# IBM/mcp-context-forge

Hardware: AMD Instinct MI355X
Metric: tool_call_req_per_s (higher is better)
Workload: dtype bf16

## Files before the change

mcp_context_forge_amd/engine.py:

```python

from __future__ import annotations

import asyncio
import json
import logging
import struct
import time
from typing import Any, Dict, List, Optional

from .config import Settings, get_settings
from .db.engine import Database
from .plugins.framework import PluginManager
from .plugins.loader import default_chain_specs, load_plugin_manager
from .protocol import jsonrpc
from .protocol.mcp import PROTOCOL_VERSION, initialize_result
from .registry.registry import NotFoundError, Registry
from .services.a2a_service import A2AService
from .services.content import CompletionService, PromptService, ResourceService, RootService
from .services.gateway_service import GatewayService
from .services.governance import CatalogService, ContentSecurity, PasswordPolicy, TokenBlocklist
from .services.llm_proxy import LLMProxyError, LLMProxyService
from .services.metrics import MetricsBuffer
from .services.observability import AuditTrail, ComplianceService, ObservabilityService, SiemExporter
from .services.sessions import CancellationService, ElicitationService, SessionRegistry
# ... 109 lines not shown
        interval = max(5.0, min(60.0, self.settings.metrics_buffer_flush_interval))
        while not self._maintenance_stop.is_set():
            try:
                await asyncio.wait_for(self._maintenance_stop.wait(), timeout=interval)
                return
            except asyncio.TimeoutError:
                pass
            try:
                self.metrics.maybe_flush()
                self.token_usage.flush()
                self.sessions.cleanup_expired()
                self.observability.flush()
                self.token_blocklist.purge_expired()
            except Exception:
                logger.exception("maintenance loop error")

    async def shutdown(self) -> None:
        if self._maintenance_task is not None:
            self._maintenance_stop.set()
            self._maintenance_task.cancel()
            try:
                await self._maintenance_task
            except (asyncio.CancelledError, Exception):
                pass
            self._maintenance_task = None
        if self.leader_elector is not None:
            await self.leader_elector.stop()
            self.leader_elector = None
        await self.gateway_service.stop()
        await self.a2a_service.aclose()
        await self.llm_proxy.aclose()
        await self.tool_service.aclose()
        await self.plugins.shutdown()
        self.observability.flush()
        self.metrics.flush()
        self.db.close()

    def enable_gpu(self) -> bool:
        if self.gpu_pipeline is not None:
            return True
        if not self.settings.gpu_enabled:
            return False
        try:
            import torch

            if not torch.cuda.is_available():
                return False
            from .gpu.pipeline import GpuPluginPipeline

            self.gpu_pipeline = GpuPluginPipeline(self)
            return True
        except Exception as exc:
            logger.warning("GPU pipeline unavailable: %s", exc)
            return False

    async def handle_rpc(self, req: jsonrpc.JSONRPCRequest, user: Optional[str] = None,
                         server_id: Optional[str] = None, session: Optional[Any] = None,
                         headers: Optional[Dict[str, str]] = None) -> Optional[jsonrpc.JSONRPCResponse]:
        method = req.method
        params = req.params if isinstance(req.params, dict) else {}
        rid = req.id
        try:
            if method == "initialize":
                if session is not None:
                    session.initialized = True
                    session.protocol_version = params.get("protocolVersion")
# ... 225 lines not shown
```

mcp_context_forge_amd/gpu/classifier.py:

```python

from __future__ import annotations

import torch

from ..models.classifier import HashedTextClassifier
from ..ops import hip


class GpuClassifier:
    def __init__(self, model: HashedTextClassifier, device: str = "cuda"):
        self.dim = model.dim
        self.hidden = model.hidden
        self.classes = model.classes
        assert self.dim % 64 == 0 and self.hidden % 128 == 0, "MFMA tile constraints"
        with torch.no_grad():
            self.w1t = model.w1.t().contiguous().to(device=device, dtype=torch.bfloat16)
            self.b1 = model.b1.to(device=device, dtype=torch.float32).contiguous()
            self.w2t = model.w2.t().contiguous().to(device=device, dtype=torch.bfloat16)
            self.b2 = model.b2.to(device=device, dtype=torch.float32).contiguous()

    def forward(self, feats_bf16: torch.Tensor) -> torch.Tensor:
        h = hip.gemm_bt(feats_bf16, self.w1t, self.b1, act=hip.ACT_GELU, out_bf16=True)
        return hip.gemv_head(h, self.w2t, self.b2, act=hip.ACT_SIGMOID)

    def forward_into(self, feats_bf16: torch.Tensor, h_buf: torch.Tensor,
                     scores_buf: torch.Tensor) -> None:
        hip.gemm_bt(feats_bf16, self.w1t, self.b1, act=hip.ACT_GELU, out_bf16=True, out=h_buf)
        hip.gemv_head(h_buf, self.w2t, self.b2, act=hip.ACT_SIGMOID, out=scores_buf)
```

mcp_context_forge_amd/gpu/pipeline.py:

```python

from __future__ import annotations

import asyncio
import json
import os
import time
import uuid
from typing import Any, Callable, Dict, List, Optional, Tuple

import numpy as np
import torch

from ..models.classifier import category_names
from ..ops import dfa, hip
from ..ops.entropy import TOL as ENTROPY_TOL
from ..ops.pybridge import get as _pb_get
from ..plugins.builtin import PII_PATTERNS, _text_of, _walk_strings
from ..plugins.framework import PluginMode
from ..protocol import jsonrpc
from ..services.upstream import InProcUpstream
from ..utils.jsonschema import validate as _validate
from .batch import pack_texts
from .classifier import GpuClassifier
from .graphs import Pass1Graphs, Pass3Graphs
# ... 73 lines not shown
                dfa.compile_patterns(
                    ["".join(ch if ch.isalnum() else "\\" + ch for ch in t) if not t.startswith("[") else t
                     for t in _NORMALIZE_TRIGGERS], case_insensitive=False), device)

        self._secret_tabs: List[Tuple[torch.Tensor, float]] = []
        if self.secrets is not None:
            tables = self.secrets.scan_tables()
            if tables is not None:
                self.banks["secrets"] = hip.DeviceScanTables(tables, device)
            self._secret_tabs = [(hip.entropy_table(tab, device), thr)
                                 for (_a, _c, tab, thr) in self.secrets.entropy_detectors]
            if not self._secret_tabs:
                self._secret_tabs = [(hip.entropy_table(np.full(256, 0xFF, dtype=np.uint8), device),
                                      float("inf"))]

        self._exfil_kw: Optional[hip.DeviceScanTables] = None
        self._exfil_tabs: List[Tuple[torch.Tensor, int]] = []
        if self.exfil is not None:
            self._exfil_kw = hip.DeviceScanTables(self.exfil.keyword_tables(), device)
            self._exfil_tabs = [(hip.entropy_table(tab, device), bits)
                                for (_e, _c, tab, bits) in self.exfil.detectors]

        self._sql_kw: Optional[hip.DeviceScanTables] = None
        self._sql_kw_len: Optional[torch.Tensor] = None
        if self.sql is not None:
            self._sql_kw = hip.DeviceScanTables(self.sql.keyword_tables(), device)
            self._sql_kw_len = torch.tensor(self.sql.keyword_lengths(), dtype=torch.int32, device=device)

        self.classifier: Optional[GpuClassifier] = None
        self.feat_dim = s.gpu_feature_dim
        if self.moderation is not None:
            self.classifier = GpuClassifier(self.moderation.model, device)
            self.feat_dim = self.moderation.dim

        self.semcache: Optional[GpuSemanticCache] = None
        if self.semcache_plugin is not None and self.semcache_plugin.cacheable_tools:
            self.semcache = GpuSemanticCache(
                capacity=max(128, (s.gpu_semcache_capacity // 128) * 128),
                dim=self.feat_dim,
                threshold=self.semcache_plugin.threshold,
                ttl_s=self.semcache_plugin.ttl,
                device=device,
                sketch_dim=s.gpu_semcache_sketch_dim,
            )

        self._pii_fixed: List[int] = []
        self._pii_active_mask = 0
        if self.pii is not None:
            fixed_index = {n: k for k, (n, _, _) in enumerate(PII_PATTERNS)}
            self._pii_fixed = [fixed_index[a[0]] for a in self.pii.active]
            self._pii_active_mask = sum(1 << i for i in self._pii_fixed)
        words = [w.lower() if self.deny.case_insensitive else w for w in self.deny.words] if self.deny else []
        self._deny_lane_ok = bool(words) and all(w.isascii() for w in words)
        self._deny_lane_blob, self._deny_lane_off = pack_strtable(words) if self._deny_lane_ok else (None, None)
        ph = [p.lower() for p in (getattr(self.harm, "phrases", None) or [])]
        self._harm_lane_ok = all(p.isascii() for p in ph)
        self._harm_lane_blob, self._harm_lane_off = pack_strtable(ph) if ph and self._harm_lane_ok else (None, None)

        self._pb = _pb_get()
        self._gpu_lock = asyncio.Lock()
        self._pin = torch.empty(16 << 20, dtype=torch.uint8, pin_memory=True)
        self._pin_off = 0

        self.banks["postmeta"] = hip.DeviceScanTables(
            dfa.compile_literals(['"structuredContent"'], case_insensitive=False), device)

# ... 319 lines not shown
            if args is BAD_ARGS:
                continue
            errs = self._schema_errors(rs.meta(j), args)
            if errs:
                rs.block(j, msg_schema(errs))
            elif hit[j]:
                rs.answer_cached(j, self._cache_result_bytes(int(hit_slot[j])))
            else:
                extra_py.append((j, args))
        return extra_py

    async def _a2a_fast_invoke(self, mt: _ToolMeta, args: Any) -> Dict[str, Any]:
        message = args.get("message") if isinstance(args, dict) else None
        if not isinstance(message, str):
            message = json.dumps(args or {}, default=str)
        t0 = time.monotonic()
        reply_text = await mt.handler(message, {})
        sc = {"agent": mt.original_name, "response": reply_text,
              "latency_ms": round((time.monotonic() - t0) * 1000, 2),
              "uaid": uuid.uuid4().hex}
        return {"content": [{"type": "text", "text": reply_text}],
                "structuredContent": sc, "isError": False}

    async def _await_gpu(self) -> None:
        ev = torch.cuda.Event()
        ev.record()
        if ev.query():
            return
        for _ in range(200000):
            await asyncio.sleep(0)
            if ev.query():
                return
        await asyncio.to_thread(ev.synchronize)

    def _upload(self, arr: np.ndarray) -> torch.Tensor:
        raw = arr.view(np.uint8).reshape(-1)
        n = raw.nbytes
        off = (self._pin_off + 255) & ~255
        if off + n > self._pin.numel():
            grow = max(self._pin.numel() * 2, off + n)
            self._pin = torch.empty(grow, dtype=torch.uint8, pin_memory=True)
            off = 0
        self._pin_off = off + n
        view = self._pin[off:off + n]
        view.numpy()[:] = raw
        cap = 1 << max(16, (n - 1).bit_length()) if n else 1
        dev = torch.empty(cap, dtype=torch.uint8, device=self.device)[:n]
        dev.copy_(view, non_blocking=True)
        tdt = {np.dtype(np.uint8): torch.uint8, np.dtype(np.int32): torch.int32,
               np.dtype(np.int64): torch.int64, np.dtype(np.float32): torch.float32}[np.dtype(arr.dtype)]
        return dev.view(tdt).reshape(arr.shape)

    async def _scan_pass(self, graphs, bankset, blob: np.ndarray, beg: np.ndarray, end: np.ndarray,
                         m: int, extra: Optional[Callable] = None, timed: bool = False):
        toc = self._toc if timed else (lambda key, t: None)
        t_g = self._tic()
        out = scores = ext = None
        await self._gpu_lock.acquire()
        try:
            toc("gp1_lockwait", t_g)
            g = graphs.get(m, int(blob.nbytes)) if graphs is not None else None
            if g is not None:
                t_st = self._tic()
                g.stage(blob, beg, end, m)
                toc("gp1_stage", t_st)
                toc("gp1_upload", t_g)
# ... 132 lines not shown
    def _pii_pass(self, obj: Any, pii_bits: int = -1) -> Tuple[Any, Optional[str]]:
        found: List[str] = []

        def fn(s: str) -> str:
            masked, f = self.pii.mask_text_subset(s, pii_bits) if pii_bits >= 0 else self.pii.mask_text(s)
            found.extend(f)
            return masked

        new = _walk_strings(obj, fn)
        if found and self.pii.action == "block" and enforcing(self.pii):
            return obj, msg_pii(found)
        return (new if found and self.pii.action == "mask" else obj), None

    async def _rewrite_pass(self, rs: RowSet, rewrite_js: List[int], hit, hit_slot,
                            pii_m, regex_m, norm_m):
        ok_items: List[Tuple[int, Any]] = []
        scan_bytes: Dict[int, bytes] = {}
        harm_c: Dict[int, int] = {}
        schema_c: Dict[int, int] = {}

        py_js = self._rewrite_native(rs, rewrite_js, pii_m, regex_m, norm_m,
                                     ok_items, scan_bytes, harm_c, schema_c)
        t_sub = self._tic()
        self._rewrite_python(rs, py_js, pii_m, regex_m, norm_m, ok_items, harm_c)
        self._toc("rw_pyloop", t_sub)
        if not ok_items:
            return None
        t_sub = self._tic()

        texts2 = [scan_bytes[j] if j in scan_bytes else _sorted_json(a).encode()
                  for (j, a) in ok_items]
        scores2_t = None
        if self.classifier is not None:
            data2, beg2, end2 = pack_texts(texts2, self.device)
            f2, _ = hip.featurize(data2, beg2, end2, self.feat_dim, pad_to=128)
            scores2_t = self.classifier.forward(f2)[: len(ok_items)]

        self._toc("rw_launch", t_sub)
        async def finish() -> List[Tuple[int, Any]]:
            return await self._finish_rewrite(rs, ok_items, harm_c, schema_c, scores2_t, hit, hit_slot)

        return finish

    def _rewrite_native(self, rs: RowSet, rewrite_js, pii_m, regex_m, norm_m,
                        ok_items, scan_bytes, harm_c, schema_c) -> List[int]:
        tools, tool_idx = rs.tools, rs.tool_idx
        rw_regex, rw_deny, rw_harm = tools.rw_regex, tools.rw_deny, tools.rw_harm
        rw_norm, rw_pii, sk_range = tools.rw_norm, tools.rw_pii, tools.sk_range
        sg_sk = enforcing(self.schema_guard) and tools.sk_tables is not None
        t_sub = self._tic()
        nat_idx: List[int] = []
        flags_l: List[int] = []
        want_l: List[int] = []
        for j in rewrite_js:
            ti = tool_idx[j]
            if regex_m[j] and rw_regex[ti]:
                continue
            deny_needed = rw_deny[ti]
            if deny_needed and not self._deny_lane_ok:
                continue
            harm_needed = rw_harm[ti]
            if harm_needed and not self._harm_lane_ok:
                continue
            do_norm = bool(norm_m[j]) and rw_norm[ti]
            do_pii = bool(pii_m[j]) and rw_pii[ti]
            fl = (1 if do_norm else 0) | (2 if do_pii else 0) | (4 if deny_needed else 0) | \
                (8 if harm_needed else 0)
            if sg_sk and sk_range[ti, 0] >= 0:
                fl |= 16
# ... 61 lines not shown

    def _rewrite_python(self, rs: RowSet, py_js, pii_m, regex_m, norm_m, ok_items, harm_c) -> None:
        tools, tool_idx = rs.tools, rs.tool_idx
        for j in py_js:
            ti = tool_idx[j]
            args = rs.decode_args(j)
            if args is BAD_ARGS:
                continue
            if self.deny is not None and tools.rw_deny[ti]:
                hay = _text_of(args)
                hay = hay.lower() if self.deny.case_insensitive else hay
                word = next((w for w in self.deny.words
                             if (w.lower() if self.deny.case_insensitive else w) in hay), None)
                if word is not None:
                    rs.block(j, msg_deny(word))
                    continue
            status, payload = self._apply_rewrites(
                tools.metas[ti].name, args, do_norm=bool(norm_m[j]), do_regex=bool(regex_m[j]),
                do_pii=bool(pii_m[j]), pii_bits=int(pii_m[j]))
            if status == "__block__":
                rs.block(j, payload)
                continue
            if self.harm is not None and tools.rw_harm[ti]:
                hay2 = _text_of(payload).lower()
                for w, ph in enumerate(self.harm.phrases):
                    if ph.lower() in hay2:
                        harm_c[j] = w
                        break
            ok_items.append((j, payload))

    async def _finish_rewrite(self, rs: RowSet, ok_items, harm_c, schema_c, scores2_t,
                              hit, hit_slot) -> List[Tuple[int, Any]]:
        t_sub = self._tic()
        if scores2_t is not None:
            await self._await_gpu()
        self._toc("rw_sync", t_sub)
        t_sub = self._tic()
        scores2 = scores2_t.cpu().numpy() if scores2_t is not None else None

        tools, tool_idx = rs.tools, rs.tool_idx
        mod_on = scores2 is not None and enforcing(self.moderation)
        sc_max = scores2.max(axis=1) if mod_on else None
        sc_arg = scores2.argmax(axis=1) if mod_on else None
        mod_thr = self.moderation.threshold if mod_on else 0.0
        cat_names = category_names(scores2.shape[1]) if mod_on else None
        sg_on = enforcing(self.schema_guard)
        mod_app, metas, harm_cats = tools.mod_app, tools.metas, (self.harm.cats if self.harm else [])

        out: List[Tuple[int, Any]] = []
        for jj, (j, args2) in enumerate(ok_items):
            ti = tool_idx[j]
            if mod_on and mod_app[ti] and float(sc_max[jj]) >= mod_thr:
                rs.block(j, msg_moderation(cat_names[int(sc_arg[jj])], float(sc_max[jj])))
                continue
            hj = harm_c.get(j, -1)
            if hj >= 0:
                rs.block(j, msg_harm(harm_cats[hj] if hj < len(harm_cats) else "?"))
                continue
            if sg_on and schema_c.get(j, 2) == 1:
                pass
            elif sg_on and metas[ti].schema_mode != "trivial":
                if isinstance(args2, bytes):
                    args2 = json.loads(args2)
                errs = self._schema_errors(metas[ti], args2)
                if errs:
                    rs.block(j, msg_schema(errs))
                    continue
            if hit[j]:
                rs.answer_cached(j, self._cache_result_bytes(int(hit_slot[j])))
                continue
            out.append((j, args2))
# ... 358 lines not shown
                result = {"content": [{"type": "text", "text": "output schema violation: " + "; ".join(errs[:3])}],
                          "isError": True}
        if enforcing(self.harm) and applies(self.harm, name):
            hay = _sorted_json(result).lower()
            for phrase, cat in zip(self.harm.phrases, self.harm.cats):
                if phrase.lower() in hay:
                    return rb, True, msg_harm(cat)
        if self.toon is not None and applies(self.toon, name) and isinstance(result, dict):
            new = self.toon.encode_result(result)
            if new is not None:
                result = new
        if self.out_guard is not None and isinstance(result, dict):
            total = sum(len(c.get("text", "")) for c in result.get("content", []) if isinstance(c, dict))
            if total > self.out_guard.max_chars and self.out_guard.action == "truncate":
                result = dict(result)
                result["content"] = [
                    {**c, "text": c["text"][: self.out_guard.max_chars]}
                    if isinstance(c, dict) and isinstance(c.get("text"), str) else c
                    for c in result.get("content", [])
                ]
        is_err = bool(isinstance(result, dict) and result.get("isError"))
        return _wire_json(result), is_err, None

    def stats(self) -> Dict[str, Any]:
        out = {
            "timing_s": {k: round(v, 4) for k, v in self.timing.items()} if self.timing_enabled else None,
            "batches": self.batches, "requests": self.requests, "fast_path": self.fast_path,
            "slow_path": self.slow_path, "blocked": self.blocked, "cache_hits": self.cache_hits,
            "host_bound": self.host_bound, "secrets_routed": self.secrets_routed,
            "exfil_routed": self.exfil_routed,
            "sql_routed": self.sql_routed,
            "post_rewrites": self.post_rewrites, "post_c": self.post_c,
            "post_c_punt": self.post_c_punt, "py_fallback": self.py_fallback,
            "banks": {k: {"states": v.n_states, "classes": v.n_classes} for k, v in self.banks.items()},
        }
        if self.semcache is not None:
            out["semcache"] = self.semcache.stats()
        return out
```

mcp_context_forge_amd/ops/build.py:

```python

from __future__ import annotations

import os
import subprocess
import sys
from pathlib import Path

CSRC = Path(__file__).parent / "csrc"
LIB = Path(__file__).parent / "libforge_hip.so"
ARCH = os.environ.get("PYTORCH_ROCM_ARCH", "gfx950")
HIPCC = os.environ.get("HIPCC", "/opt/rocm/bin/hipcc")

SOURCES = ["scan.hip", "entropy.hip", "exfil.hip", "sql.hip", "featurize.hip", "json_guard.hip", "gemm_bf16.hip",
           "runtime.hip", "gemm_v2.hip", "envelope.cpp", "upstream.cpp", "fastpath.cpp", "rewrite.cpp", "pool.cpp"]


PYBRIDGE = Path(__file__).parent / "forge_pybridge.so"
EDGE = Path(__file__).parent / "forge_edge.so"
HEY = Path(__file__).parent / "forge_hey"


def needs_build() -> bool:
    if not LIB.exists():
        return True
    lib_mtime = LIB.stat().st_mtime
    watched = [CSRC / f for f in SOURCES] + sorted(CSRC.glob("*.h"))
    return any(f.stat().st_mtime > lib_mtime for f in watched)


def build_pybridge(force: bool = False, verbose: bool = True) -> Path:
    src = CSRC / "pybridge.c"
    if not force and PYBRIDGE.exists() and PYBRIDGE.stat().st_mtime > src.stat().st_mtime:
        return PYBRIDGE
    import sysconfig

    cc = os.environ.get("CC", "gcc")
    cmd = [cc, "-O2", "-fPIC", "-shared", f"-I{sysconfig.get_paths()['include']}",
           "-o", str(PYBRIDGE), str(src)]
    if verbose:
        print("[forge-pybridge]", " ".join(cmd), file=sys.stderr)
    subprocess.run(cmd, check=True)
    return PYBRIDGE


def build_edge(force: bool = False, verbose: bool = True) -> Path:
    src = CSRC / "edge.cpp"
    newest = max(src.stat().st_mtime, (CSRC / "edge_pack.hpp").stat().st_mtime)
# ... 51 lines not shown
```

mcp_context_forge_amd/ops/csrc/forge_api.h:

```cpp
#ifndef FORGE_API_H
#define FORGE_API_H

#include <stdint.h>

#define FORGE_ACT_NONE 0
#define FORGE_ACT_GELU 1
#define FORGE_ACT_SIGMOID 2

#define FORGE_ERR_SHAPE 9001
#define FORGE_ERR_ACT 9002
#define FORGE_ERR_GEMV_K 9003
#define FORGE_ERR_ROW_ALIGN 9004
#define FORGE_ERR_DECODE_SCAN 9005
#define FORGE_ERR_SQL_SCAN 9006

#define FORGE_SCAN_LDS_LIMIT (64 * 1024)
#define FORGE_SCAN_TABLE_BYTES(n_states, n_classes) \
    ((int64_t)(n_states) * (n_classes) * 2 + 256 + (int64_t)(n_states) * 4)

#define FORGE_DECODE_SCAN_TABLE_LIMIT (16 * 1024)
#define FORGE_DECODE_SCAN_KW_MAX_LEN 16

#define FORGE_SQL_SCAN_TABLE_LIMIT (16 * 1024)
#define FORGE_SQL_SCAN_MIN_KW 6
#define FORGE_SQL_SCAN_MAX_KW 29
#define FORGE_SQL_SCAN_KW_MAX_LEN 16

typedef void (*forge_task_fn)(int index, void* ctx);

#ifdef __cplusplus
extern "C" {
#endif


int forge_scan(const void* data, const void* beg, const void* end_, int batch,
               const void* next, const void* klass, const void* accept,
               int n_states, int n_classes,
               void* out_mask, void* out_first_end, void* stream);

int forge_scan_multi(const void* data, const void* beg, const void* end_, int batch,
                     const void* descs_dev, int n_banks, int lds_bytes,
                     void* out_mask, void* stream);

int forge_token_entropy(const void* data, const void* beg, const void* end_, int batch,
                        const void* sym, int min_len,
                        void* out_h, void* out_span, void* out_runs, void* out_flags,
                        void* stream);

int forge_decode_scan(const void* data, const void* beg, const void* end_, int batch,
                      const void* sym, int bits, int min_len, int min_printable_permille,
                      const void* next, const void* klass, const void* accept,
                      int n_states, int n_classes, int kw_max_len,
                      void* out_counts, void* out_kw, void* out_span, void* out_flags,
                      void* stream);

int forge_sql_scan(const void* data, const void* beg, const void* end_, int batch,
                   const void* next, const void* klass, const void* accept,
                   int n_states, int n_classes, const void* kw_len, int n_kw, int kw_max_len,
                   int dquote_boundary,
                   void* out_counts, void* out_blocked, void* out_first, void* out_flags,
                   void* stream);

int forge_featurize(const void* data, const void* beg, const void* end_, int batch, int dim,
                    void* out_bf16, void* out_f32, void* stream);

int forge_json_guard(const void* data, const void* beg, const void* end_, int batch,
                     int max_depth, int max_string,
                     void* out_status, void* out_depth, void* stream);

int forge_gemm_bt(const void* A, const void* BT, const void* bias, void* C,
                  int M, int N, int K, int act, int out_bf16, void* stream);

int forge_gemm_bt_v2(const void* A, const void* BT, const void* bias, void* C,
                     int M, int N, int K, int act, int out_bf16, void* stream);

int forge_gemv_head(const void* A, const void* WT, const void* bias, void* out,
                    int M, int C, int K, int act, void* stream);

int forge_rows_argmax_merge(const void* scores, int M, int Nc, int idx_base, const void* valid,
                            void* best_val, void* best_idx, void* stream);

int forge_rows_gather_scatter_bf16(const void* src, const void* src_rows, const void* dst_slots,
                                   void* dst, void* valid, int R, int D, void* stream);

int forge_verify_dot(const void* feats, const void* keys, const void* idx, void* out,
                     int M, int D, void* stream);


void forge_parallel_for(int n, forge_task_fn fn, void* ctx);

int forge_parse_envelopes(const uint8_t* data, const int64_t* offsets, int n,
                          int32_t* kind, int32_t* id_beg, int32_t* id_end,
                          int32_t* name_beg, int32_t* name_end,
                          int32_t* args_beg, int32_t* args_end);

int64_t forge_upstream_call_batch(const uint8_t* data, const int32_t* args_beg,
                                  const int32_t* args_end, const int32_t* kinds, int n,
                                  const char* now_iso, uint8_t* out, int64_t out_cap,
                                  int64_t* res_beg, int64_t* res_end);

void* forge_store_new(int capacity);

void forge_store_put(void* store, int slot, const uint8_t* data, int64_t n);

void forge_store_put_batch(void* store, const int32_t* slots, int n,
                           const uint8_t* blob, const int64_t* beg, const int64_t* end);

int64_t forge_store_get(void* store, int slot, uint8_t* out, int64_t cap);

void forge_store_free(void* store);

void* forge_cache_new(double ttl);

void forge_cache_free(void* cache);

void* forge_toolmap_new(const uint8_t* blob, const int32_t* beg, const int32_t* end, int nt);

void forge_toolmap_free(void* map);

// ... 62 lines not shown
```

mcp_context_forge_amd/ops/hip.py:

```python

from __future__ import annotations

import ctypes
import os
from functools import lru_cache
from typing import List, Optional, Tuple

import numpy as np
import torch

from . import entropy, exfil, sql
from .dfa import ScanTables


class ForgeHipError(RuntimeError):
    pass


_KINDS = {"p": ctypes.c_void_p, "s": ctypes.c_char_p, "i": ctypes.c_int, "u": ctypes.c_uint32,
          "l": ctypes.c_int64, "d": ctypes.c_double, "v": None}


def _sig(ret: str, args: str):
    return _KINDS[ret], [_KINDS[c] for c in args.replace(" ", "")]


_API = {
    "forge_scan": _sig("i", "ppp i ppp ii pp p"),
    "forge_scan_multi": _sig("i", "ppp i p ii p p"),
    "forge_token_entropy": _sig("i", "ppp i pi pppp p"),
    "forge_decode_scan": _sig("i", "ppp i piii ppp iii pppp p"),
    "forge_sql_scan": _sig("i", "ppp i ppp ii pii i pppp p"),
    "forge_featurize": _sig("i", "ppp ii pp p"),
    "forge_json_guard": _sig("i", "ppp i ii pp p"),
    "forge_gemm_bt": _sig("i", "pppp iii ii p"),
    "forge_gemm_bt_v2": _sig("i", "pppp iii ii p"),
    "forge_gemv_head": _sig("i", "pppp iii i p"),
    "forge_rows_argmax_merge": _sig("i", "p iii p pp p"),
    "forge_rows_gather_scatter_bf16": _sig("i", "ppp p p ii p"),
    "forge_verify_dot": _sig("i", "ppp p ii p"),
    "forge_parallel_for": _sig("v", "i p p"),
    "forge_parse_envelopes": _sig("i", "pp i p pp pp pp"),
    "forge_upstream_call_batch": _sig("l", "ppp p i s p l pp"),
    "forge_store_new": _sig("p", "i"),
    "forge_store_put": _sig("v", "p i p l"),
    "forge_store_put_batch": _sig("v", "p p i p pp"),
    "forge_store_get": _sig("l", "p i p l"),
    "forge_store_free": _sig("v", "p"),
    "forge_cache_new": _sig("p", "d"),
    "forge_cache_free": _sig("v", "p"),
    "forge_toolmap_new": _sig("p", "ppp i"),
    "forge_toolmap_free": _sig("v", "p"),
    "forge_toolmap_resolve": _sig("v", "p p pp i p"),
    "forge_decide": _sig("l", "p pp pp p pp pppppp ppp pp p i ppp ppp p u ppi ppi ppi pp d ppp pl pp"),
    "forge_finalize": _sig("l", "p pp pp p p i pi ppp p ppp p p dd pl pp pp"),
    "forge_rewrite_rows": _sig("l", "ppp i pp u i ii pp ii ppp pl pp pp pp i p ppp pp pp p"),
    "forge_post_rows": _sig("l", "ppp i p u i pp i l d pppp pl pp"),
}


@lru_cache(maxsize=1)
def _load() -> ctypes.CDLL:
    from .build import LIB, build

    if not LIB.exists():
        build()
    lib = ctypes.CDLL(str(LIB))
    for name, (restype, argtypes) in _API.items():
        fn = getattr(lib, name)
        fn.restype = restype
        fn.argtypes = argtypes
    return lib

# ... 59 lines not shown


def scan_table_bytes(n_states: int, n_classes: int) -> int:
    return n_states * n_classes * 2 + 256 + n_states * 4


class ScanBankSet:

    def __init__(self, banks: List[Tuple[str, "DeviceScanTables"]], device: str = "cuda"):
        self.names = [n for n, _ in banks]
        self.banks = [b for _, b in banks]
        self.n = len(self.banks)
        self.index = {n: i for i, n in enumerate(self.names)}
        self.lds_bytes = 0
        recs = np.zeros((max(self.n, 1), 6), dtype=np.int64)
        for i, b in enumerate(self.banks):
            tbytes = scan_table_bytes(b.n_states, b.n_classes)
            use_lds = 1 if tbytes <= SCAN_LDS_LIMIT else 0
            if use_lds:
                self.lds_bytes = max(self.lds_bytes, tbytes)
            recs[i, 0] = b.next.data_ptr()
            recs[i, 1] = b.klass.data_ptr()
            recs[i, 2] = b.accept.data_ptr()
            recs[i, 3] = (b.n_states & 0xFFFFFFFF) | (b.n_classes << 32)
            recs[i, 4] = use_lds
        self.descs = torch.from_numpy(recs).to(device)


def scan_multi(data: torch.Tensor, beg: torch.Tensor, end: torch.Tensor,
               bankset: ScanBankSet, out: Optional[torch.Tensor] = None) -> torch.Tensor:
    batch = beg.numel()
    if out is None:
        out = torch.zeros((bankset.n, batch), dtype=torch.int32, device=data.device)
    else:
        out.zero_()
    if bankset.n == 0 or batch == 0:
        return out
    _check("forge_scan_multi", _load().forge_scan_multi(
        _ptr(data), _ptr(beg), _ptr(end), batch,
        _ptr(bankset.descs), bankset.n, bankset.lds_bytes,
        _ptr(out), _stream()))
    return out


ENTROPY_BASE64 = entropy.base64_table
ENTROPY_HEX = entropy.hex_table


def entropy_table(sym_table, device: str = "cuda") -> torch.Tensor:
    t = np.ascontiguousarray(np.asarray(sym_table, dtype=np.uint8).reshape(-1))
    if t.shape[0] != 256:
        raise ValueError("symbol table must have 256 entries")
    return torch.from_numpy(t.copy()).to(device)


def token_entropy(data: torch.Tensor, beg: torch.Tensor, end: torch.Tensor, sym_table,
                  min_len: int, out: Optional[Tuple[torch.Tensor, ...]] = None
                  ) -> Tuple[torch.Tensor, torch.Tensor, torch.Tensor, torch.Tensor]:
    batch = beg.numel()
    if not isinstance(sym_table, torch.Tensor):
        sym_table = entropy_table(sym_table, str(data.device))
    if sym_table.dtype != torch.uint8 or sym_table.numel() != 256:
        raise ValueError("symbol table must be uint8[256]")
    if out is None:
        dev = data.device
        out = (torch.empty(batch, dtype=torch.float32, device=dev),
               torch.empty((batch, 2), dtype=torch.int32, device=dev),
# ... 85 lines not shown
               max_string: int = 1 << 20) -> Tuple[torch.Tensor, torch.Tensor]:
    batch = beg.numel()
    status = torch.zeros(batch, dtype=torch.int32, device=data.device)
    depth = torch.zeros(batch, dtype=torch.int32, device=data.device)
    _check("forge_json_guard", _load().forge_json_guard(
        _ptr(data), _ptr(beg), _ptr(end), batch, max_depth, max_string, _ptr(status), _ptr(depth), _stream()))
    return status, depth


ACT_NONE, ACT_GELU, ACT_SIGMOID = 0, 1, 2


def gemm_bt(a: torch.Tensor, bt: torch.Tensor, bias: Optional[torch.Tensor] = None,
            act: int = ACT_NONE, out_bf16: bool = False,
            out: Optional[torch.Tensor] = None) -> torch.Tensor:
    assert a.dtype == torch.bfloat16 and bt.dtype == torch.bfloat16
    assert a.is_contiguous() and bt.is_contiguous()
    m, k = a.shape
    n, k2 = bt.shape
    assert k == k2, (a.shape, bt.shape)
    if out is None:
        out = torch.empty((m, n), dtype=torch.bfloat16 if out_bf16 else torch.float32, device=a.device)
    if m % 256 == 0 and n % 256 == 0 and k % 32 == 0 and not os.environ.get("FORGE_GEMM_V1"):
        rc = _load().forge_gemm_bt_v2(_ptr(a), _ptr(bt), _ptr(bias), _ptr(out), m, n, k,
                                      act, 1 if out_bf16 else 0, _stream())
        _check("forge_gemm_bt_v2", rc)
        return out
    rc = _load().forge_gemm_bt(_ptr(a), _ptr(bt), _ptr(bias), _ptr(out), m, n, k,
                               act, 1 if out_bf16 else 0, _stream())
    _check("forge_gemm_bt", rc)
    return out


def gemv_head(a: torch.Tensor, wt: torch.Tensor, bias: Optional[torch.Tensor] = None,
              act: int = ACT_NONE, out: Optional[torch.Tensor] = None) -> torch.Tensor:
    m, k = a.shape
    c, k2 = wt.shape
    assert k == k2 and c <= 32
    if out is None:
        out = torch.empty((m, c), dtype=torch.float32, device=a.device)
    _check("forge_gemv_head", _load().forge_gemv_head(_ptr(a), _ptr(wt), _ptr(bias), _ptr(out), m, c, k, act, _stream()))
    return out


def rows_argmax_merge(scores: torch.Tensor, best_val: torch.Tensor, best_idx: torch.Tensor,
                      idx_base: int = 0, valid: Optional[torch.Tensor] = None) -> None:
    m, nc = scores.shape
    _check("forge_rows_argmax_merge", _load().forge_rows_argmax_merge(
        _ptr(scores), m, nc, idx_base, _ptr(valid), _ptr(best_val), _ptr(best_idx), _stream()))


def rows_gather_scatter_bf16(src: torch.Tensor, src_rows: torch.Tensor, dst_slots: torch.Tensor,
                             dst: torch.Tensor, valid: Optional[torch.Tensor] = None) -> None:
    r = src_rows.numel()
    d = src.shape[1]
    _check("forge_rows_gather_scatter_bf16", _load().forge_rows_gather_scatter_bf16(
        _ptr(src), _ptr(src_rows), _ptr(dst_slots), _ptr(dst), _ptr(valid), r, d, _stream()))


def verify_dot(feats: torch.Tensor, keys: torch.Tensor, idx: torch.Tensor) -> torch.Tensor:
    m, d = feats.shape
    out = torch.empty(m, dtype=torch.float32, device=feats.device)
    _check("forge_verify_dot", _load().forge_verify_dot(
        _ptr(feats), _ptr(keys), _ptr(idx), _ptr(out), m, d, _stream()))
    return out



ENV_NEEDS_PY, ENV_PARSE_ERR, ENV_OTHER, ENV_TOOLS_CALL = -2, -1, 0, 1


def parse_envelopes(blob: np.ndarray, offsets: np.ndarray) -> dict:
    n = offsets.shape[0] - 1
    kind = np.empty(n, dtype=np.int32)
    id_b = np.empty(n, dtype=np.int32)
    id_e = np.empty(n, dtype=np.int32)
    nm_b = np.empty(n, dtype=np.int32)
    nm_e = np.empty(n, dtype=np.int32)
    ar_b = np.empty(n, dtype=np.int32)
    ar_e = np.empty(n, dtype=np.int32)

    p = _np_ptr
    _check("forge_parse_envelopes", _load().forge_parse_envelopes(
        p(blob), p(offsets), n, p(kind), p(id_b), p(id_e), p(nm_b), p(nm_e), p(ar_b), p(ar_e)))
    return {"kind": kind, "id_beg": id_b, "id_end": id_e,
            "name_beg": nm_b, "name_end": nm_e, "args_beg": ar_b, "args_end": ar_e}


def upstream_call_batch(blob: np.ndarray, args_beg: np.ndarray, args_end: np.ndarray,
                        kinds: np.ndarray, now_iso: str) -> Tuple[np.ndarray, np.ndarray, np.ndarray]:
    n = kinds.shape[0]
    res_b = np.empty(n, dtype=np.int64)
    res_e = np.empty(n, dtype=np.int64)

    lib, p = _load(), _np_ptr
    spans_total = int((args_end[kinds >= 0] - np.maximum(args_beg[kinds >= 0], 0)).clip(min=0).sum()) if n else 0
    cap = spans_total * 3 + n * 256 + 1024
    out = np.empty(cap, dtype=np.uint8)
# ... 210 lines not shown
```

Baseline: 300,600.

## Add native rescore session with pinned slots and skinny GEMM for rewrite moderation

The rewrite-path moderation rescore moves into a native C/HIP session. It packs the texts into pinned per-slot arenas, issues one H2D copy, runs featurize, GEMM and GEMV on the stream, copies the scores back asynchronously and records an event. This replaces the Python pack_texts/featurize/torch forward path and its blocking .cpu() readback. A new 64x64-tile skinny MFMA GEMM kernel is added for small-M batches, and scan_multi no longer zeroes a preallocated output buffer. The change adds slot-management complexity and can fall back to the eager path when every slot is busy.

Result: faster. 347,800, median of 6 (+15.7%).

```diff
diff --git a/mcp_context_forge_amd/engine.py b/mcp_context_forge_amd/engine.py
--- a/mcp_context_forge_amd/engine.py
+++ b/mcp_context_forge_amd/engine.py
@@ -165,6 +165,8 @@
         await self.llm_proxy.aclose()
         await self.tool_service.aclose()
         await self.plugins.shutdown()
+        if self.gpu_pipeline is not None:
+            self.gpu_pipeline.close()
         self.observability.flush()
         self.metrics.flush()
         self.db.close()
diff --git a/mcp_context_forge_amd/gpu/classifier.py b/mcp_context_forge_amd/gpu/classifier.py
--- a/mcp_context_forge_amd/gpu/classifier.py
+++ b/mcp_context_forge_amd/gpu/classifier.py
@@ -5,6 +5,9 @@
 
 from ..models.classifier import HashedTextClassifier
 from ..ops import hip
+
+
+SKINNY_MAX_M = 4096
 
 
 class GpuClassifier:
@@ -19,11 +22,18 @@
             self.w2t = model.w2.t().contiguous().to(device=device, dtype=torch.bfloat16)
             self.b2 = model.b2.to(device=device, dtype=torch.float32).contiguous()
 
+    def _gemm(self, m: int):
+        if m <= SKINNY_MAX_M and hip.gemm_skinny_enabled() and hip.gemm_skinny_fits(m, self.hidden, self.dim):
+            return hip.gemm_bt_skinny
+        return hip.gemm_bt
+
     def forward(self, feats_bf16: torch.Tensor) -> torch.Tensor:
-        h = hip.gemm_bt(feats_bf16, self.w1t, self.b1, act=hip.ACT_GELU, out_bf16=True)
+        gemm = self._gemm(feats_bf16.shape[0])
+        h = gemm(feats_bf16, self.w1t, self.b1, act=hip.ACT_GELU, out_bf16=True)
         return hip.gemv_head(h, self.w2t, self.b2, act=hip.ACT_SIGMOID)
 
     def forward_into(self, feats_bf16: torch.Tensor, h_buf: torch.Tensor,
                      scores_buf: torch.Tensor) -> None:
-        hip.gemm_bt(feats_bf16, self.w1t, self.b1, act=hip.ACT_GELU, out_bf16=True, out=h_buf)
+        gemm = self._gemm(feats_bf16.shape[0])
+        gemm(feats_bf16, self.w1t, self.b1, act=hip.ACT_GELU, out_bf16=True, out=h_buf)
         hip.gemv_head(h_buf, self.w2t, self.b2, act=hip.ACT_SIGMOID, out=scores_buf)
diff --git a/mcp_context_forge_amd/gpu/pipeline.py b/mcp_context_forge_amd/gpu/pipeline.py
--- a/mcp_context_forge_amd/gpu/pipeline.py
+++ b/mcp_context_forge_amd/gpu/pipeline.py
@@ -129,6 +129,11 @@
         if self.moderation is not None:
             self.classifier = GpuClassifier(self.moderation.model, device)
             self.feat_dim = self.moderation.dim
+        self._rescore: Optional[hip.RescoreSession] = None
+        if self.classifier is not None:
+            c = self.classifier
+            self._rescore = hip.RescoreSession(c.w1t, c.b1, c.w2t, c.b2)
+        self.rescore_native = self.rescore_eager = 0
 
         self.semcache: Optional[GpuSemanticCache] = None
         if self.semcache_plugin is not None and self.semcache_plugin.cacheable_tools:
@@ -514,6 +519,33 @@
             if ev.query():
                 return
         await asyncio.to_thread(ev.synchronize)
+
+    def _rescore_submit(self, texts: List[bytes]) -> int:
+        sess = self._rescore
+        if sess is None or os.environ.get("FORGE_RESCORE_NATIVE", "1") == "0":
+            return -1
+        blob, offs = self._pb.concat_with_offsets(texts)
+        slot = sess.submit(blob, offs, len(texts))
+        return slot if slot >= 0 else -1
+
+    async def _rescore_collect(self, slot: int, n: int) -> np.ndarray:
+        sess = self._rescore
+        try:
+            if not sess.poll(slot):
+                for _ in range(200000):
+                    await asyncio.sleep(0)
+                    if sess.poll(slot):
+                        break
+                else:
+                    await asyncio.to_thread(sess.wait, slot)
+            return sess.scores(slot, n)
+        finally:
+            sess.release(slot)
+
+    def close(self) -> None:
+        sess, self._rescore = self._rescore, None
+        if sess is not None:
+            sess.close()
 
     def _upload(self, arr: np.ndarray) -> torch.Tensor:
         raw = arr.view(np.uint8).reshape(-1)
@@ -712,9 +744,15 @@
                   for (j, a) in ok_items]
         scores2_t = None
         if self.classifier is not None:
-            data2, beg2, end2 = pack_texts(texts2, self.device)
-            f2, _ = hip.featurize(data2, beg2, end2, self.feat_dim, pad_to=128)
-            scores2_t = self.classifier.forward(f2)[: len(ok_items)]
+            slot = self._rescore_submit(texts2)
+            if slot >= 0:
+                scores2_t = slot
+                self.rescore_native += 1
+            else:
+                data2, beg2, end2 = pack_texts(texts2, self.device)
+                f2, _ = hip.featurize(data2, beg2, end2, self.feat_dim, pad_to=128)
+                scores2_t = self.classifier.forward(f2)[: len(ok_items)]
+                self.rescore_eager += 1
 
         self._toc("rw_launch", t_sub)
         async def finish() -> List[Tuple[int, Any]]:
@@ -842,11 +880,16 @@
     async def _finish_rewrite(self, rs: RowSet, ok_items, harm_c, schema_c, scores2_t,
                               hit, hit_slot) -> List[Tuple[int, Any]]:
         t_sub = self._tic()
-        if scores2_t is not None:
-            await self._await_gpu()
-        self._toc("rw_sync", t_sub)
-        t_sub = self._tic()
-        scores2 = scores2_t.cpu().numpy() if scores2_t is not None else None
+        if isinstance(scores2_t, int):
+            scores2 = await self._rescore_collect(scores2_t, len(ok_items))
+            self._toc("rw_sync", t_sub)
+            t_sub = self._tic()
+        else:
+            if scores2_t is not None:
+                await self._await_gpu()
+            self._toc("rw_sync", t_sub)
+            t_sub = self._tic()
+            scores2 = scores2_t.cpu().numpy() if scores2_t is not None else None
 
         tools, tool_idx = rs.tools, rs.tool_idx
         mod_on = scores2 is not None and enforcing(self.moderation)
@@ -1271,6 +1314,7 @@
             "sql_routed": self.sql_routed,
             "post_rewrites": self.post_rewrites, "post_c": self.post_c,
             "post_c_punt": self.post_c_punt, "py_fallback": self.py_fallback,
+            "rescore_native": self.rescore_native, "rescore_eager": self.rescore_eager,
             "banks": {k: {"states": v.n_states, "classes": v.n_classes} for k, v in self.banks.items()},
         }
         if self.semcache is not None:
diff --git a/mcp_context_forge_amd/ops/build.py b/mcp_context_forge_amd/ops/build.py
--- a/mcp_context_forge_amd/ops/build.py
+++ b/mcp_context_forge_amd/ops/build.py
@@ -12,7 +12,7 @@
 HIPCC = os.environ.get("HIPCC", "/opt/rocm/bin/hipcc")
 
 SOURCES = ["scan.hip", "entropy.hip", "exfil.hip", "sql.hip", "featurize.hip", "json_guard.hip", "gemm_bf16.hip",
-           "runtime.hip", "gemm_v2.hip", "envelope.cpp", "upstream.cpp", "fastpath.cpp", "rewrite.cpp", "pool.cpp"]
+           "runtime.hip", "gemm_v2.hip", "gemm_skinny.hip", "rescore.hip", "envelope.cpp", "upstream.cpp", "fastpath.cpp", "rewrite.cpp", "pool.cpp"]
 
 
 PYBRIDGE = Path(__file__).parent / "forge_pybridge.so"
diff --git a/mcp_context_forge_amd/ops/csrc/forge_api.h b/mcp_context_forge_amd/ops/csrc/forge_api.h
--- a/mcp_context_forge_amd/ops/csrc/forge_api.h
+++ b/mcp_context_forge_amd/ops/csrc/forge_api.h
@@ -13,6 +13,8 @@
 #define FORGE_ERR_ROW_ALIGN 9004
 #define FORGE_ERR_DECODE_SCAN 9005
 #define FORGE_ERR_SQL_SCAN 9006
+#define FORGE_ERR_RESCORE_ARGS 9007
+#define FORGE_ERR_RESCORE_BUSY 9008
 
 #define FORGE_SCAN_LDS_LIMIT (64 * 1024)
 #define FORGE_SCAN_TABLE_BYTES(n_states, n_classes) \
@@ -74,6 +76,9 @@
 int forge_gemm_bt_v2(const void* A, const void* BT, const void* bias, void* C,
                      int M, int N, int K, int act, int out_bf16, void* stream);
 
+int forge_gemm_bt_skinny(const void* A, const void* BT, const void* bias, void* C,
+                         int M, int N, int K, int act, int out_bf16, void* stream);
+
 int forge_gemv_head(const void* A, const void* WT, const void* bias, void* out,
                     int M, int C, int K, int act, void* stream);
 
@@ -85,6 +90,22 @@
 
 int forge_verify_dot(const void* feats, const void* keys, const void* idx, void* out,
                      int M, int D, void* stream);
+
+void* forge_rescore_new(const void* w1t, const void* b1, const void* w2t, const void* b2,
+                        int dim, int hidden, int classes,
+                        int max_rows, int64_t max_bytes, int n_slots);
+
+int forge_rescore_submit(void* ctx, const uint8_t* blob, const int64_t* offs, int n, void* stream);
+
+int forge_rescore_poll(void* ctx, int slot);
+
+int forge_rescore_wait(void* ctx, int slot);
+
+const float* forge_rescore_scores(void* ctx, int slot);
+
+void forge_rescore_release(void* ctx, int slot);
+
+void forge_rescore_free(void* ctx);
 
 
 void forge_parallel_for(int n, forge_task_fn fn, void* ctx);
diff --git a/mcp_context_forge_amd/ops/csrc/gemm_skinny.hip b/mcp_context_forge_amd/ops/csrc/gemm_skinny.hip
--- /dev/null
+++ b/mcp_context_forge_amd/ops/csrc/gemm_skinny.hip
@@ -0,0 +1,138 @@
+
+#include "gemm_common.h"
+
+#define SK_BM 64
+#define SK_BN 64
+#define SK_BK 64
+#define SK_ROWB (SK_BK * 2)
+#define SK_SLOT_A (SK_BM * SK_ROWB)
+#define SK_SLOT_B (SK_BN * SK_ROWB)
+#define SK_RING 4
+#define SK_AHEAD 3
+
+__device__ __forceinline__ uint32_t swz_sk(uint32_t byte_off) {
+    return byte_off ^ (((byte_off >> 7) & 7u) << 4);
+}
+
+template <int ACT, bool OUT_BF16, bool HAS_BIAS>
+__global__ __launch_bounds__(256, 2) void gemm_bt_skinny_kernel(
+    const short* __restrict__ A,
+    const short* __restrict__ BT,
+    const float* __restrict__ bias,
+    void* __restrict__ C,
+    int M, int N, int K)
+{
+    __shared__ short lds[SK_RING * (SK_SLOT_A + SK_SLOT_B) / 2];
+    char* lds_a = (char*)lds;
+    char* lds_b = (char*)lds + SK_RING * SK_SLOT_A;
+
+    const int tid = threadIdx.x;
+    const int lane = tid & (WAVE - 1);
+    const int wave = tid >> 6;
+    const int wm = wave >> 1;
+    const int wn = wave & 1;
+    const int tile_m = blockIdx.x * SK_BM;
+    const int tile_n = blockIdx.y * SK_BN;
+    const int n_tiles = K / SK_BK;
+
+    f32x4 acc[2][2];
+    #pragma unroll
+    for (int i = 0; i < 2; ++i)
+        #pragma unroll
+        for (int j = 0; j < 2; ++j)
+            acc[i][j] = (f32x4){0.f, 0.f, 0.f, 0.f};
+
+    auto stage_tile = [&](int t) {
+        const int slot = t & (SK_RING - 1);
+        #pragma unroll
+        for (int i = 0; i < 2; ++i) {
+            uint32_t P = (uint32_t)(i * 256 + tid) * 16u;
+            uint32_t L = swz_sk(P);
+            uint32_t row = L >> 7, colb = L & 127u;
+            const short* gA = A + ((size_t)(tile_m + row) * K + t * SK_BK) + (colb >> 1);
+            __builtin_amdgcn_global_load_lds(
+                (const __attribute__((address_space(1))) uint32_t*)gA,
+                (__attribute__((address_space(3))) uint32_t*)(lds_a + (size_t)slot * SK_SLOT_A
+                                                              + (i * 256 + (wave * 64)) * 16),
+                16, 0, 0);
+        }
+        #pragma unroll
+        for (int i = 0; i < 2; ++i) {
+            uint32_t P = (uint32_t)(i * 256 + tid) * 16u;
+            uint32_t L = swz_sk(P);
+            uint32_t row = L >> 7, colb = L & 127u;
+            const short* gB = BT + ((size_t)(tile_n + row) * K + t * SK_BK) + (colb >> 1);
+            __builtin_amdgcn_global_load_lds(
+                (const __attribute__((address_space(1))) uint32_t*)gB,
+                (__attribute__((address_space(3))) uint32_t*)(lds_b + (size_t)slot * SK_SLOT_B
+                                                              + (i * 256 + (wave * 64)) * 16),
+                16, 0, 0);
+        }
+    };
+    auto wait_tiles = [&](int ahead) {
+        if (ahead >= 2) asm volatile("s_waitcnt vmcnt(8)" ::: "memory");
+        else if (ahead == 1) asm volatile("s_waitcnt vmcnt(4)" ::: "memory");
+        else asm volatile("s_waitcnt vmcnt(0)" ::: "memory");
+    };
+
+    #pragma unroll
+    for (int t = 0; t < SK_AHEAD; ++t)
+        if (t < n_tiles) stage_tile(t);
+    wait_tiles(min(SK_AHEAD, n_tiles) - 1);
+    __builtin_amdgcn_s_barrier();
+
+    const uint32_t k_col = (uint32_t)((lane >> 4) * 16);
+    const uint32_t a_row_base = (uint32_t)(wm * 32 + (lane & 15));
+    const uint32_t b_row_base = (uint32_t)(wn * 32 + (lane & 15));
+
+    for (int kt = 0; kt < n_tiles; ++kt) {
+        const char* slot_a = lds_a + (size_t)(kt & (SK_RING - 1)) * SK_SLOT_A;
+        const char* slot_b = lds_b + (size_t)(kt & (SK_RING - 1)) * SK_SLOT_B;
+
+        if (kt + SK_AHEAD < n_tiles) stage_tile(kt + SK_AHEAD);
+
+        #pragma unroll
+        for (int kk = 0; kk < 2; ++kk) {
+            bf16x8 a_frag[2], b_frag[2];
+            #pragma unroll
+            for (int f = 0; f < 2; ++f) {
+                uint32_t ra = a_row_base + f * 16, rb = b_row_base + f * 16;
+                a_frag[f] = *(const bf16x8*)(slot_a + swz_sk(ra * SK_ROWB + kk * 64 + k_col));
+                b_frag[f] = *(const bf16x8*)(slot_b + swz_sk(rb * SK_ROWB + kk * 64 + k_col));
+            }
+            #pragma unroll
+            for (int fr = 0; fr < 2; ++fr)
+                #pragma unroll
+                for (int fc = 0; fc < 2; ++fc)
+                    acc[fr][fc] = __builtin_amdgcn_mfma_f32_16x16x32_bf16(a_frag[fr], b_frag[fc], acc[fr][fc], 0, 0, 0);
+        }
+        if (kt + 1 < n_tiles) {
+            wait_tiles(min(kt + SK_AHEAD, n_tiles - 1) - (kt + 1));
+            __builtin_amdgcn_s_barrier();
+        }
+    }
+
+    #pragma unroll
+    for (int fr = 0; fr < 2; ++fr) {
+        #pragma unroll
+        for (int fc = 0; fc < 2; ++fc) {
+            int col = tile_n + wn * 32 + fc * 16 + (lane & 15);
+            int row0 = tile_m + wm * 32 + fr * 16 + (lane >> 4) * 4;
+            store_frag<ACT, OUT_BF16, HAS_BIAS>(acc[fr][fc], bias, C, N, row0, col);
+        }
+    }
+}
+
+extern "C" int forge_gemm_bt_skinny(
+    const void* A, const void* BT, const void* bias, void* C,
+    int M, int N, int K, int act, int out_bf16, void* stream)
+{
+    if (M <= 0 || N <= 0 || K <= 0 || (M % SK_BM) || (N % SK_BN) || (K % SK_BK)) return FORGE_ERR_SHAPE;
+    hipStream_t s = (hipStream_t)stream;
+    dim3 grid(M / SK_BM, N / SK_BN);
+    return dispatch_epilogue(act, out_bf16 != 0, bias != nullptr, [&](auto e) {
+        using E = decltype(e);
+        hipLaunchKernelGGL((gemm_bt_skinny_kernel<E::act, E::out_bf16, E::has_bias>), grid, dim3(256), 0, s,
+                           (const short*)A, (const short*)BT, (const float*)bias, C, M, N, K);
+    });
+}
diff --git a/mcp_context_forge_amd/ops/csrc/rescore.hip b/mcp_context_forge_amd/ops/csrc/rescore.hip
--- /dev/null
+++ b/mcp_context_forge_amd/ops/csrc/rescore.hip
@@ -0,0 +1,186 @@
+
+#include "common.h"
+
+#include <stdlib.h>
+#include <string.h>
+
+#include <new>
+
+namespace {
+
+enum : int { SLOT_FREE = 0, SLOT_BUSY = 1, SLOT_DRAINING = 2 };
+
+struct RescoreSlot {
+    uint8_t* pin_arena = nullptr;
+    uint8_t* dev_arena = nullptr;
+    short* feats = nullptr;
+    short* h = nullptr;
+    float* scores = nullptr;
+    float* pin_scores = nullptr;
+    hipEvent_t done = nullptr;
+    int state = SLOT_FREE;
+};
+
+struct RescoreSession {
+    const void* w1t; const void* b1; const void* w2t; const void* b2;
+    int dim, hidden, classes, max_rows, rows_cap, n_slots;
+    int64_t max_bytes, bytes_off;
+    bool skinny;
+    RescoreSlot* slots;
+};
+
+int round_up(int v, int m) { return (v + m - 1) / m * m; }
+
+void free_session(RescoreSession* s) {
+    if (s == nullptr) return;
+    for (int i = 0; s->slots != nullptr && i < s->n_slots; ++i) {
+        RescoreSlot& sl = s->slots[i];
+        if (sl.done) { (void)hipEventSynchronize(sl.done); (void)hipEventDestroy(sl.done); }
+        if (sl.pin_arena) (void)hipHostFree(sl.pin_arena);
+        if (sl.pin_scores) (void)hipHostFree(sl.pin_scores);
+        if (sl.dev_arena) (void)hipFree(sl.dev_arena);
+        if (sl.feats) (void)hipFree(sl.feats);
+        if (sl.h) (void)hipFree(sl.h);
+        if (sl.scores) (void)hipFree(sl.scores);
+    }
+    delete[] s->slots;
+    delete s;
+}
+
+}
+
+extern "C" void* forge_rescore_new(
+    const void* w1t, const void* b1, const void* w2t, const void* b2,
+    int dim, int hidden, int classes, int max_rows, int64_t max_bytes, int n_slots)
+{
+    if (max_rows <= 0) max_rows = 1024;
+    if (max_bytes <= 0) max_bytes = (int64_t)512 * max_rows;
+    if (n_slots <= 0) n_slots = 4;
+    if (w1t == nullptr || w2t == nullptr || dim < 64 || (dim & (dim - 1)) || hidden <= 0 ||
+        (hidden % 128) || (hidden % (WAVE * 8)) || classes <= 0 || classes > 32 ||
+        max_bytes > ((int64_t)1 << 30))
+        return nullptr;
+
+    RescoreSession* s = new (std::nothrow) RescoreSession();
+    if (s == nullptr) return nullptr;
+    s->w1t = w1t; s->b1 = b1; s->w2t = w2t; s->b2 = b2;
+    s->dim = dim; s->hidden = hidden; s->classes = classes;
+    s->max_rows = max_rows; s->rows_cap = round_up(max_rows, 128);
+    s->n_slots = n_slots; s->max_bytes = max_bytes;
+    s->bytes_off = ((int64_t)(max_rows + 1) * 4 + 15) & ~(int64_t)15;
+    const char* env = getenv("FORGE_GEMM_SKINNY");
+    s->skinny = !(env != nullptr && env[0] == '0' && env[1] == '\0');
+    s->slots = new (std::nothrow) RescoreSlot[n_slots];
+    if (s->slots == nullptr) { delete s; return nullptr; }
+
+    const size_t arena = (size_t)(s->bytes_off + max_bytes);
+    const size_t feats_b = (size_t)s->rows_cap * dim * 2;
+    bool ok = true;
+    for (int i = 0; ok && i < n_slots; ++i) {
+        RescoreSlot& sl = s->slots[i];
+        ok = hipHostMalloc((void**)&sl.pin_arena, arena, hipHostMallocDefault) == hipSuccess
+          && hipHostMalloc((void**)&sl.pin_scores, (size_t)max_rows * classes * 4, hipHostMallocDefault) == hipSuccess
+          && hipMalloc((void**)&sl.dev_arena, arena) == hipSuccess
+          && hipMalloc((void**)&sl.feats, feats_b) == hipSuccess
+          && hipMalloc((void**)&sl.h, (size_t)s->rows_cap * hidden * 2) == hipSuccess
+          && hipMalloc((void**)&sl.scores, (size_t)s->rows_cap * classes * 4) == hipSuccess
+          && hipMemset(sl.feats, 0, feats_b) == hipSuccess
+          && hipEventCreateWithFlags(&sl.done, hipEventDisableTiming) == hipSuccess;
+    }
+    if (!ok) { (void)hipGetLastError(); free_session(s); return nullptr; }
+    return s;
+}
+
+extern "C" int forge_rescore_submit(void* ctx, const uint8_t* blob, const int64_t* offs, int n, void* stream)
+{
+    RescoreSession* s = (RescoreSession*)ctx;
+    if (s == nullptr || blob == nullptr || offs == nullptr || n <= 0 || n > s->max_rows)
+        return -FORGE_ERR_RESCORE_ARGS;
+    const int64_t base = offs[0];
+    if (base < 0) return -FORGE_ERR_RESCORE_ARGS;
+    for (int i = 0; i < n; ++i)
+        if (offs[i + 1] < offs[i]) return -FORGE_ERR_RESCORE_ARGS;
+    const int64_t total = offs[n] - base;
+    if (total > s->max_bytes) return -FORGE_ERR_RESCORE_ARGS;
+
+    int slot = -1;
+    for (int i = 0; i < s->n_slots && slot < 0; ++i) {
+        RescoreSlot& sl = s->slots[i];
+        if (sl.state == SLOT_DRAINING && hipEventQuery(sl.done) == hipSuccess) sl.state = SLOT_FREE;
+        if (sl.state == SLOT_FREE) slot = i;
+    }
+    (void)hipGetLastError();
+    if (slot < 0) return -FORGE_ERR_RESCORE_BUSY;
+    RescoreSlot& sl = s->slots[slot];
+    hipStream_t st = (hipStream_t)stream;
+
+    int32_t* o32 = (int32_t*)sl.pin_arena;
+    for (int i = 0; i <= n; ++i) o32[i] = (int32_t)(offs[i] - base);
+    memcpy(sl.pin_arena + s->bytes_off, blob + base, (size_t)total);
+
+    int rc = (int)hipMemcpyAsync(sl.dev_arena, sl.pin_arena, (size_t)(s->bytes_off + total),
+                                 hipMemcpyHostToDevice, st);
+    if (rc != 0) return -rc;
+    const int32_t* d_offs = (const int32_t*)sl.dev_arena;
+    rc = forge_featurize(sl.dev_arena + s->bytes_off, d_offs, d_offs + 1, n, s->dim, sl.feats, nullptr, stream);
+    if (rc == 0) {
+        if (s->skinny)
+            rc = forge_gemm_bt_skinny(sl.feats, s->w1t, s->b1, sl.h, round_up(n, 64), s->hidden, s->dim,
+                                      FORGE_ACT_GELU, 1, stream);
+        else
+            rc = forge_gemm_bt(sl.feats, s->w1t, s->b1, sl.h, round_up(n, 128), s->hidden, s->dim,
+                               FORGE_ACT_GELU, 1, stream);
+    }
+    if (rc == 0)
+        rc = forge_gemv_head(sl.h, s->w2t, s->b2, sl.scores, n, s->classes, s->hidden, FORGE_ACT_SIGMOID, stream);
+    if (rc == 0)
+        rc = (int)hipMemcpyAsync(sl.pin_scores, sl.scores, (size_t)n * s->classes * 4, hipMemcpyDeviceToHost, st);
+    int rc_ev = (int)hipEventRecord(sl.done, st);
+    if (rc != 0 || rc_ev != 0) {
+        sl.state = SLOT_DRAINING;
+        return -(rc != 0 ? rc : rc_ev);
+    }
+    sl.state = SLOT_BUSY;
+    return slot;
+}
+
+static RescoreSlot* rescore_slot(void* ctx, int slot) {
+    RescoreSession* s = (RescoreSession*)ctx;
+    if (s == nullptr || slot < 0 || slot >= s->n_slots) return nullptr;
+    return &s->slots[slot];
+}
+
+extern "C" int forge_rescore_poll(void* ctx, int slot)
+{
+    RescoreSlot* sl = rescore_slot(ctx, slot);
+    if (sl == nullptr || sl->state != SLOT_BUSY) return -FORGE_ERR_RESCORE_ARGS;
+    hipError_t e = hipEventQuery(sl->done);
+    if (e == hipSuccess) return 1;
+    if (e == hipErrorNotReady) { (void)hipGetLastError(); return 0; }
+    return -(int)e;
+}
+
+extern "C" int forge_rescore_wait(void* ctx, int slot)
+{
+    RescoreSlot* sl = rescore_slot(ctx, slot);
+    if (sl == nullptr || sl->state != SLOT_BUSY) return -FORGE_ERR_RESCORE_ARGS;
+    hipError_t e = hipEventSynchronize(sl->done);
+    return e == hipSuccess ? 1 : -(int)e;
+}
+
+extern "C" const float* forge_rescore_scores(void* ctx, int slot)
+{
+    RescoreSlot* sl = rescore_slot(ctx, slot);
+    return sl != nullptr ? sl->pin_scores : nullptr;
+}
+
+extern "C" void forge_rescore_release(void* ctx, int slot)
+{
+    RescoreSlot* sl = rescore_slot(ctx, slot);
+    if (sl != nullptr && sl->state == SLOT_BUSY) sl->state = SLOT_DRAINING;
+}
+
+extern "C" void forge_rescore_free(void* ctx)
+{
+    free_session((RescoreSession*)ctx);
+}
diff --git a/mcp_context_forge_amd/ops/hip.py b/mcp_context_forge_amd/ops/hip.py
--- a/mcp_context_forge_amd/ops/hip.py
+++ b/mcp_context_forge_amd/ops/hip.py
@@ -35,10 +35,18 @@
     "forge_json_guard": _sig("i", "ppp i ii pp p"),
     "forge_gemm_bt": _sig("i", "pppp iii ii p"),
     "forge_gemm_bt_v2": _sig("i", "pppp iii ii p"),
+    "forge_gemm_bt_skinny": _sig("i", "pppp iii ii p"),
     "forge_gemv_head": _sig("i", "pppp iii i p"),
     "forge_rows_argmax_merge": _sig("i", "p iii p pp p"),
     "forge_rows_gather_scatter_bf16": _sig("i", "ppp p p ii p"),
     "forge_verify_dot": _sig("i", "ppp p ii p"),
+    "forge_rescore_new": _sig("p", "pppp iii i l i"),
+    "forge_rescore_submit": _sig("i", "p ss i p"),
+    "forge_rescore_poll": _sig("i", "p i"),
+    "forge_rescore_wait": _sig("i", "p i"),
+    "forge_rescore_scores": _sig("p", "p i"),
+    "forge_rescore_release": _sig("v", "p i"),
+    "forge_rescore_free": _sig("v", "p"),
     "forge_parallel_for": _sig("v", "i p p"),
     "forge_parse_envelopes": _sig("i", "pp i p pp pp pp"),
     "forge_upstream_call_batch": _sig("l", "ppp p i s p l pp"),
@@ -164,7 +172,7 @@
     batch = beg.numel()
     if out is None:
         out = torch.zeros((bankset.n, batch), dtype=torch.int32, device=data.device)
-    else:
+    elif bankset.n == 0:
         out.zero_()
     if bankset.n == 0 or batch == 0:
         return out
@@ -316,6 +324,35 @@
     return out
 
 
+ERR_SHAPE = 9001
+
+SKINNY_TILE = 64
+
+
+def gemm_skinny_enabled() -> bool:
+    return os.environ.get("FORGE_GEMM_SKINNY", "1") != "0"
+
+
+def gemm_skinny_fits(m: int, n: int, k: int) -> bool:
+    return m > 0 and n > 0 and k > 0 and m % SKINNY_TILE == 0 and n % SKINNY_TILE == 0 \
+        and k % SKINNY_TILE == 0
+
+
+def gemm_bt_skinny(a: torch.Tensor, bt: torch.Tensor, bias: Optional[torch.Tensor] = None,
+                   act: int = ACT_NONE, out_bf16: bool = False,
+                   out: Optional[torch.Tensor] = None) -> torch.Tensor:
+    assert a.dtype == torch.bfloat16 and bt.dtype == torch.bfloat16
+    assert a.is_contiguous() and bt.is_contiguous()
+    m, k = a.shape
+    n, k2 = bt.shape
+    assert k == k2, (a.shape, bt.shape)
+    if out is None:
+        out = torch.empty((m, n), dtype=torch.bfloat16 if out_bf16 else torch.float32, device=a.device)
+    _check("forge_gemm_bt_skinny", _load().forge_gemm_bt_skinny(
+        _ptr(a), _ptr(bt), _ptr(bias), _ptr(out), m, n, k, act, 1 if out_bf16 else 0, _stream()))
+    return out
+
+
 def gemv_head(a: torch.Tensor, wt: torch.Tensor, bias: Optional[torch.Tensor] = None,
               act: int = ACT_NONE, out: Optional[torch.Tensor] = None) -> torch.Tensor:
     m, k = a.shape
@@ -348,6 +385,69 @@
     _check("forge_verify_dot", _load().forge_verify_dot(
         _ptr(feats), _ptr(keys), _ptr(idx), _ptr(out), m, d, _stream()))
     return out
+
+
+ERR_RESCORE_ARGS, ERR_RESCORE_BUSY = 9007, 9008
+
+
+class RescoreSession:
+
+    def __init__(self, w1t: torch.Tensor, b1: torch.Tensor, w2t: torch.Tensor, b2: torch.Tensor,
+                 max_rows: int = 1024, max_bytes: int = 0, n_slots: int = 4):
+        assert w1t.dtype == torch.bfloat16 and w2t.dtype == torch.bfloat16
+        assert b1.dtype == torch.float32 and b2.dtype == torch.float32
+        assert all(t.is_contiguous() for t in (w1t, b1, w2t, b2))
+        self._weights = (w1t, b1, w2t, b2)
+        self.hidden, self.dim = w1t.shape
+        self.classes = w2t.shape[0]
+        self.max_rows = max_rows
+        self.max_bytes = max_bytes if max_bytes > 0 else 512 * max_rows
+        self.n_slots = n_slots
+        self._lib = _load()
+        with torch.cuda.device(w1t.device):
+            ctx = self._lib.forge_rescore_new(_ptr(w1t), _ptr(b1), _ptr(w2t), _ptr(b2),
+                                              self.dim, self.hidden, self.classes,
+                                              max_rows, self.max_bytes, n_slots)
+        if not ctx:
+            raise ForgeHipError("forge_rescore_new failed")
+        self._ctx = ctypes.c_void_p(ctx)
+        self._scores = []
+        for slot in range(n_slots):
+            ptr = self._lib.forge_rescore_scores(self._ctx, slot)
+            buf = (ctypes.c_float * (max_rows * self.classes)).from_address(ptr)
+            self._scores.append(np.frombuffer(buf, dtype=np.float32).reshape(max_rows, self.classes))
+
+    def submit(self, blob: bytes, offs: bytes, n: int) -> int:
+        return self._lib.forge_rescore_submit(self._ctx, blob, offs, n, _stream())
+
+    def poll(self, slot: int) -> bool:
+        rc = self._lib.forge_rescore_poll(self._ctx, slot)
+        if rc < 0:
+            raise ForgeHipError(f"forge_rescore_poll failed with code {-rc}")
+        return rc == 1
+
+    def wait(self, slot: int) -> None:
+        rc = self._lib.forge_rescore_wait(self._ctx, slot)
+        if rc < 0:
+            raise ForgeHipError(f"forge_rescore_wait failed with code {-rc}")
+
+    def scores(self, slot: int, n: int) -> np.ndarray:
+        return self._scores[slot][:n].copy()
+
+    def release(self, slot: int) -> None:
+        self._lib.forge_rescore_release(self._ctx, slot)
+
+    def close(self) -> None:
+        if self._ctx is not None:
+            self._scores = []
+            self._lib.forge_rescore_free(self._ctx)
+            self._ctx = None
+
+    def __del__(self):
+        try:
+            self.close()
+        except Exception:
+            pass
 
 
 
```
